# oleg-savchenko/jax_nbody_emulator_with_dj

Hardware: AMD Instinct MI355X
Metric: voxels/sec (disp+vel) on 512^3 box, ndiv=4 (higher is better)
Workload: dtype f32-equivalent: f16x3 split MFMA (3 f16 MFMAs per product, f32 accumulate)

## Files before the change

jax_nbody_emulator_with_dj_amd/csrc/nbe_engine_internal.h:

```cpp
#pragma once

#include "../../include/nbe.h"
#include "nbe_kernels.h"

#include <cmath>
#include <cstdarg>
#include <cstdio>
#include <cstdlib>
#include <cstring>
#include <algorithm>
#include <atomic>
#include <chrono>
#include <condition_variable>
#include <deque>
#include <functional>
#include <map>
#include <memory>
#include <mutex>
#include <string>
#include <thread>
#include <vector>

#pragma GCC visibility push(hidden)

// ... 184 lines not shown
    uint64_t graph_clock = 0, graph_replays = 0;
    int epoch = 0;
    hipEvent_t ev_g0 = nullptr, ev_g1 = nullptr;
    struct Probe {
        bool on = false, tile = false;
        int p[3] = {0, 0, 0}, nout = 0;
        int o[3] = {0, 0, 0};
        struct Slot { std::string name; int C, n, nw, level; int64_t off; };
        std::vector<Slot> slots;
        unsigned* bits = nullptr; int64_t words = 0;
        unsigned* count = nullptr;
    } probe;
    int* paths = nullptr;
    bool prof = false;
    std::vector<ProfEntry> prof_entries;
    struct Pending { int entry; hipEvent_t a, b; };
    std::vector<Pending> pending;
    std::vector<hipEvent_t> ev_pool;
};

struct HeadOut { void* disp; void* velo; int out_dtype; int OD, OH, OW, a0, a1, a2; float Dz, vel_fac; };

static constexpr int PIPE_EDGE = 32;

static constexpr int BRICK_H1 = 6, BRICK_H2 = 10;
static constexpr int BRICK_H0 = 4;

bool is_device_ptr(const void* p);
int require_ready(nbe_ctx* c);
int prepare_range(nbe_ctx* c, const float* dev_src, int64_t n, float Dz, const float* host_src = nullptr);
int check_range(nbe_ctx* c);

int planes_for(int C, int prec);
Tensor talloc(nbe_ctx* c, int C, int D, int H, int W);
Tensor tallocp(nbe_ctx* c, int C, int D, int Hi, int Wi, int pad);
void fill_halo(nbe_ctx* c, const Tensor& t);
void tfree(nbe_ctx* c, Tensor& t);
Tensor zview(const Tensor& t, int z0, int nz);
void set_org(Tensor& t, int z, int y, int x);
bool wino_f16_layer(int prec, bool vel, int cin_pad);
bool wino_env_off();
bool up8_launch(const nbe_ctx* c, const Layer& L, bool has_dx);
int run_conv(nbe_ctx* c, const Layer& L, const ConvLaunch& cl_in, bool has_dx);
const Layer* find_layer(nbe_ctx* c, const char* block, const char* layer);
bool block_fused(const nbe_ctx* c, const Layer* L1, int nres);
bool two_source_width(const nbe_ctx* c);
Tensor alloc_hidden(nbe_ctx* c, int cmid, int nz, const Tensor& x, bool fused);
int resblock_part(nbe_ctx* c, const char* name, const Tensor& x, const Tensor& h, const Tensor& s,
                  int js, int ns, int jh, int nh, bool has_dx, bool final_act, const int* zr, const Tensor* x2 = nullptr);
int resblock(nbe_ctx* c, const char* name, const Tensor& x, bool has_dx, bool final_act, int cout, int cmid, Tensor* out,
             Tensor* hidden_out = nullptr);
int down_conv(nbe_ctx* c, const Layer& L, const Tensor& x, Tensor& o, bool probe);
int downblock(nbe_ctx* c, const char* name, const Tensor& x, Tensor* out);
int upblock(nbe_ctx* c, const char* name, const Tensor& x, const Tensor& cat, int xcrop = 0, int g0 = -1);
void crop_into(nbe_ctx* c, const Tensor& src, int crop, const Tensor& dst, int cz = -1);
int check_dims(int D, int H, int W);
int check_dims_pyx(int D, int H, int W);
void run_head(nbe_ctx* c, const Tensor& y, const Tensor& xin, const HeadOut& h, int zoff);
int network(nbe_ctx* c, const Tensor& tin, Tensor* yout);
int network_stream(nbe_ctx* c, const Tensor& tin, const HeadOut& ho, int S);

PackedW layer_geometry(int prec, int kind, int cout, int cin);
bool packs_narrow(int prec, bool vel, const Layer& L);
bool packs_wino(int prec, bool vel, const Layer& L);
bool packs_wino_skip(int prec, bool vel, bool style, const Layer& L);
bool packs_stem(int prec, const Layer& L);
int alloc_wino(PackedW& pw);
int alloc_stem(PackedW& pw);
int wino_flag_round_trip(nbe_ctx* c, const std::function<void()>& packs);
void release_layer(Layer& L);
void free_layers(nbe_ctx* c);
int pack_wino(nbe_ctx* c);

unsigned host_absmax_bits(const float* x, int64_t n);
int pipe_input(nbe_ctx* c, const Tensor& tin, int t0, int t1, int look, float scale);
int pipe_output(nbe_ctx* c, int z, int n, int a1 = 0, int a2 = 0, int e1 = -1, int e2 = -1);
int ensure_workspace(nbe_ctx* c, int D, int H, int W);
int run_subbox(nbe_ctx* c, const float* box, int Db, int Hb, int Wb, int o0, int o1, int o2,
               int D, int H, int W, float Dz, float vel_fac, void* disp, void* velo, int out_dtype,
               int OD, int OH, int OW, int a0, int a1, int a2);
void drop_graphs(nbe_ctx* c);
int64_t plan_budget(nbe_ctx* c, int64_t reserve);
int choose_slab(nbe_ctx* c, int D, int H, int W, int64_t budget, int64_t* need_out, bool pyx = false, bool pz = false);

void brick_send(nbe_ctx* c, const Tensor& t, int in, int n, void* lo, void* hi);
// ... 13 lines not shown
```

jax_nbody_emulator_with_dj_amd/csrc/nbe_engine_net.cpp:

```cpp
#include "nbe_engine_internal.h"

int planes_for(int C, int prec) { return roundup(C, 16) / (prec == PREC_F16 ? 8 : 4); }

static Planes ws_planes(nbe_ctx* c, int G, int D, int H, int W, int64_t* off_out) {
    Planes p;
    p.G = G; p.D = D; p.H = H; p.W = W;
    p.pstride = (p.vox() + 63) & ~int64_t(63);
    const int64_t one = (int64_t)G * p.pstride * 16;
    const int64_t slack = ((int64_t)2 * H * W + 2 * W + 1024) * 16;
    const int64_t off = c->arena.alloc(one * (c->vel ? 2 : 1) + slack);
    *off_out = off;
    if (!c->dry) {
        p.x = (float*)(c->ws + off);
        p.dx = c->vel ? (float*)(c->ws + off + one) : nullptr;
    }
    return p;
}

Tensor talloc(nbe_ctx* c, int C, int D, int H, int W) {
    Tensor t;
    t.p = ws_planes(c, planes_for(C, c->prec), D, H, W, &t.off);
    const int gw = c->prec == PREC_F16 ? (C + 7) / 8 : c->prec == PREC_F16X3 ? 2 * ((C + 7) / 8) : (C + 3) / 4;
    if (!c->dry && t.off >= 0 && gw < t.p.G) {
        const size_t off = (size_t)gw * t.p.pstride * 4, bytes = (size_t)(t.p.G - gw) * t.p.pstride * 16;
        launch_zero(t.p.x + off, (int64_t)bytes, c->stream);
        if (t.p.dx) launch_zero(t.p.dx + off, (int64_t)bytes, c->stream);
    }
    return t;
}
Tensor tallocp(nbe_ctx* c, int C, int D, int Hi, int Wi, int pad) {
    Tensor t = talloc(c, C, D, Hi + 2 * pad, Wi + 2 * pad);
    t.pad = pad;
    return t;
}
static Planes inner(const Tensor& t) {
    Planes p = t.p;
    const int64_t sh = (int64_t)t.pad * (t.p.W + 1) * 4;
    if (p.x) p.x += sh;
    if (p.dx) p.dx += sh;
    return p;
}
void fill_halo(nbe_ctx* c, const Tensor& t) {
    if (t.pad > 0 && !c->dry) launch_fill_yx(t.p, t.pad, c->vel, c->stream);
}
void tfree(nbe_ctx* c, Tensor& t) { if (t.off >= 0) c->arena.release(t.off); t.off = -1; }
Tensor zview(const Tensor& t, int z0, int nz) {
    Tensor v = t;
    v.off = -1;
    const int64_t sh = (int64_t)z0 * t.p.H * t.p.W * 4;
    if (v.p.x) v.p.x += sh;
    if (v.p.dx) v.p.dx += sh;
    v.p.D = nz;
    v.org[0] += z0;
    return v;
}
static void org_conv(const Tensor& x, int nconv, int out[3]) {
    const int p = x.pad ? nconv : 0;
    out[0] = x.org[0]; out[1] = x.org[1] - p; out[2] = x.org[2] - p;
}
void set_org(Tensor& t, int z, int y, int x) { t.org[0] = z; t.org[1] = y; t.org[2] = x; }

static std::string conv_name(const PackedW& pw, bool vel, bool has_dx, bool g6 = false, bool up8 = false) {
    if (up8) return vel ? "up_h3<8 parities,vel,dx>" : "up_h3<8 parities,novel>";
    const char* m = pw.mode == MODE_FLAT3 ? "FLAT3" : pw.mode == MODE_FLAT1 ? "FLAT1" : "DOWN";
// ... 33 lines not shown
    int pe = -1; hipEvent_t ea = nullptr, eb = nullptr;
    if (c->prof) {
        std::string pn = cl.wino ? std::string(c->prec == PREC_F16 ? "conv_h1w<FLAT3,vel,dx>" : c->vel ? "conv_h3w<FLAT3,vel,dx>" : "conv_h3w<FLAT3,novel>")
                                 : conv_name(pw, c->vel, has_dx, g6, cl.set < 0);
        static const bool per_layer = getenv("NBE_PROF_LAYERS") && atoi(getenv("NBE_PROF_LAYERS")) == 1;
        if (per_layer) pn += " " + L.block + "/" + L.layer;
        pe = prof_entry(c, pn);
        ea = get_event(c); eb = get_event(c);
        (void)hipEventRecord(ea, c->stream);
    }
    if (launch_conv(pw, cl, c->vel, has_dx, c->stream))
        return fail("internal error: no kernel for layer %s/%s (mode %d, gauged %d, input tangent %d, crop offset %ld, output stride %d)",
                    L.block.c_str(), L.layer.c_str(), L.pw.mode, (int)g6, (int)has_dx, (long)cl.in_off, cl.osz);
    if (c->prof) {
        (void)hipEventRecord(eb, c->stream);
        c->pending.push_back({pe, ea, eb});
        const double nout = (double)cl.Dv * cl.Hv * cl.Wv * (cl.set < 0 ? 8.0 : 1.0);
        const int taps = L.kind == 0 ? 27 : L.kind == 2 ? 8 : 1;
        const double gemms = c->vel ? ((has_dx && !g6) ? 3.0 : 2.0) : 1.0;
        c->prof_entries[pe].flops += 2.0 * nout * L.cout * L.cin * taps * gemms;
        if (cl.skw) c->prof_entries[pe].flops += 2.0 * nout * L.cout * L.fskip->cin * (!c->vel ? 1.0 : (cl.flags & F_SKIP_NODX) ? 2.0 : 3.0);
        c->prof_entries[pe].launches += 1;
        if (c->pending.size() > 4096) prof_collect(c);
    }
    return 0;
}

const Layer* find_layer(nbe_ctx* c, const char* block, const char* layer) {
    auto it = c->layers.find(std::string(block) + "/" + layer);
    return it == c->layers.end() ? nullptr : &it->second;
}


static bool wino_only_fuse(const nbe_ctx* c) { return !c->vel || c->prec == PREC_F16; }
bool block_fused(const nbe_ctx* c, const Layer* L1, int nres) {
    return c->fuse && L1->fskip != nullptr && (!wino_only_fuse(c) || (!c->direct_z && !wino_env_off() && (nres & 1) == 0));
}

bool two_source_width(const nbe_ctx* c) { return c->mid % (c->prec == PREC_F16 ? 32 : 16) == 0; }

Tensor alloc_hidden(nbe_ctx* c, int cmid, int nz, const Tensor& x, bool fused) {
    const int pad = x.pad, sy = pad ? 0 : 2;
    if (fused && !pad) return talloc(c, cmid, nz, x.p.H, x.p.W);
    return tallocp(c, cmid, nz, x.p.H - 2 * pad - sy, x.p.W - 2 * pad - sy, pad);
}

int resblock_part(nbe_ctx* c, const char* name, const Tensor& x, const Tensor& h, const Tensor& s,
                         int js, int ns, int jh, int nh, bool has_dx, bool final_act, const int* zr, const Tensor* x2) {
    const Layer *Ls = find_layer(c, name, "skip"), *L0 = find_layer(c, name, "conv_0"), *L1 = find_layer(c, name, "conv_1");
    if (!Ls || !L0 || !L1) return fail("missing layers of block %s", name);
    const int H = x.p.H, W = x.p.W, pad = x.pad;
    const bool fused = block_fused(c, L1, ns);
    if (fused && (h.p.H != H || h.p.W != W)) return fail("internal: hidden tensor of fused block %s lacks the input's pitch", name);
    if (x2 && (!fused || x2->p.H != H || x2->p.W != W || x2->pad != pad)) return fail("internal: two-source input of block %s", name);
    const Tensor sv = zview(s, js, ns), hv = zview(h, jh, nh);
    const Tensor xs = zview(x, js, ns + 4);
    const int64_t sk_off = (2L * H + (pad ? pad : 2)) * W + (pad ? pad : 2);
    if (!fused) {
        ConvLaunch cl; cl.in = xs.p; cl.in_off = sk_off;
        cl.Dv = ns; cl.Hv = s.p.H - 2 * pad; cl.Wv = s.p.W - 2 * pad; cl.out = inner(sv); cl.flags = 0;
        if (run_conv(c, *Ls, cl, has_dx)) return 1;
    }
    int og[3];
    {
        ConvLaunch cl; cl.in = zview(x, jh, nh + 2).p; cl.Dv = nh; cl.Hv = H - 2; cl.Wv = W - 2; cl.out = inner(hv); cl.flags = F_ACT;
        if (x2) { cl.in2 = zview(*x2, jh, nh + 2).p; cl.csplit_ch = c->mid; }
        if (run_conv(c, *L0, cl, has_dx)) return 1;
        org_conv(x, 1, og); og[0] += jh;
        const int zh[3] = {zr ? zr[0] : 0, zr ? zr[1] + 2 : 0, zr ? zr[2] : 0};
        probe_act(c, *L0, cl.out, 0, og, cl.Dv, cl.Hv, cl.Wv, pad != 0, zr ? zh : nullptr);
    }
    fill_halo(c, hv);
    {
        ConvLaunch cl; cl.in = zview(h, js, ns + 2).p; cl.Dv = ns; cl.Hv = s.p.H - 2 * pad; cl.Wv = s.p.W - 2 * pad; cl.out = inner(sv);
        if (fused) { cl.sk = xs.p; cl.sk_off = sk_off; cl.skw = L1->pwn.w ? &Ls->pwn : &Ls->pw; cl.flags = (final_act ? F_ACT : 0) | (has_dx ? 0 : F_SKIP_NODX);
                     if (x2) { cl.sk2 = zview(*x2, js, ns + 4).p; cl.sk_split_ch = c->mid; } }
        else { cl.res = inner(sv); cl.flags = F_RES | (final_act ? F_ACT : 0); }
        if (run_conv(c, *L1, cl, true)) return 1;
        org_conv(x, 2, og); og[0] += js;
        if (final_act) probe_act(c, *L1, cl.out, 0, og, cl.Dv, cl.Hv, cl.Wv, pad != 0, zr);
    }
    fill_halo(c, sv);
    return 0;
}

int resblock(nbe_ctx* c, const char* name, const Tensor& x, bool has_dx, bool final_act, int cout, int cmid, Tensor* out,
                    Tensor* hidden_out) {
    const Layer* L1 = find_layer(c, name, "conv_1");
    if (!L1) return fail("missing layers of block %s", name);
    const int D = x.p.D, pad = x.pad;
    const int sy = pad ? 0 : 2;
    Tensor s = tallocp(c, cout, D - 4, x.p.H - 2 * pad - 2 * sy, x.p.W - 2 * pad - 2 * sy, pad);
    Tensor h = alloc_hidden(c, cmid, D - 2, x, block_fused(c, L1, D - 4));
    if (s.off < 0 || h.off < 0) return fail("workspace exhausted in block %s", name);
    if (resblock_part(c, name, x, h, s, 0, D - 4, 0, D - 2, has_dx, final_act, nullptr)) return 1;
    tfree(c, h);
    if (hidden_out) *hidden_out = h;
    int og[3];
    org_conv(x, 2, og);
    set_org(s, og[0], og[1], og[2]);
    *out = s;
    return 0;
}

static void carry_planes(nbe_ctx* c, const Tensor& t, int src, int dst, int n) {
    if (c->dry || n <= 0) return;
    launch_crop(zview(t, src, n).p, 0, zview(t, dst, n).p, 0, c->vel, c->stream, 0);
}

int down_conv(nbe_ctx* c, const Layer& L, const Tensor& x, Tensor& o, bool probe) {
    ConvLaunch cl; cl.in = inner(x); cl.Dv = o.p.D; cl.Hv = o.p.H; cl.Wv = o.p.W; cl.out = o.p; cl.flags = F_ACT;
    if (run_conv(c, L, cl, true)) return 1;
    set_org(o, x.org[0] / 2, x.org[1] / 2, x.org[2] / 2);
    if (probe) probe_act(c, L, cl.out, 0, o.org, cl.Dv, cl.Hv, cl.Wv, x.pad != 0);
    return 0;
}

int downblock(nbe_ctx* c, const char* name, const Tensor& x, Tensor* out) {
    const Layer* L = find_layer(c, name, "conv_0");
    if (!L) return fail("missing layer %s/conv_0", name);
    Tensor o = talloc(c, c->mid, x.p.D / 2, x.p.H / 2, x.p.W / 2);
    if (o.off < 0) return fail("workspace exhausted in %s", name);
    if (down_conv(c, *L, x, o, true)) return 1;
    *out = o;
    return 0;
}

static int mid_planes(const nbe_ctx* c) { return c->mid / (c->prec == PREC_F16 ? 8 : 4); }

int upblock(nbe_ctx* c, const char* name, const Tensor& x, const Tensor& cat, int xcrop, int g0) {
    const Layer* L = find_layer(c, name, "conv_0");
    if (!L) return fail("missing layer %s/conv_0", name);
    xcrop += x.pad;
    const int Hx = x.p.H - 2 * xcrop, Wx = x.p.W - 2 * xcrop;
    if (cat.p.D != 2 * x.p.D || cat.p.H - 2 * cat.pad != 2 * Hx || cat.p.W - 2 * cat.pad != 2 * Wx)
        return fail("internal: concat geometry mismatch in %s", name);
    const bool up8 = up8_launch(c, *L, true);
    const int out_g0 = g0 >= 0 ? g0 : mid_planes(c);
    for (int p = 0; p < (up8 ? 1 : 8); ++p) {
        ConvLaunch cl; cl.in = x.p; cl.in_off = ((int64_t)xcrop * x.p.W + xcrop);
        cl.Dv = x.p.D; cl.Hv = Hx; cl.Wv = Wx; cl.out = inner(cat);
        cl.out_g0 = out_g0; cl.osz = 2; cl.oz = (p >> 2) & 1; cl.oy = (p >> 1) & 1; cl.ox = p & 1;
        cl.flags = F_ACT; cl.set = up8 ? -1 : p;
        if (run_conv(c, *L, cl, true)) return 1;
    }
    const int xc = xcrop - x.pad;
    const int og[3] = {2 * x.org[0], 2 * (x.org[1] + xc), 2 * (x.org[2] + xc)};
    probe_act(c, *L, inner(cat), out_g0, og, 2 * x.p.D, 2 * Hx, 2 * Wx, cat.pad != 0);
// ... 4 lines not shown
    if (c->dry) return;
    Planes s = src.p; s.G = mid_planes(c);
    launch_crop(s, crop, dst.p, 0, c->vel, c->stream, cz);
}

int check_dims(int D, int H, int W) {
    const int v[3] = {D, H, W};
    for (int i = 0; i < 3; ++i)
        if (v[i] < 104 || v[i] % 8 != 0)
            return fail("input spatial size %d unsupported: each of (D,H,W) must be >= 104 and a multiple of 8 "
                        "(all-VALID U-Net with three 2x levels, receptive-field crop 48)", v[i]);
    return 0;
}

void run_head(nbe_ctx* c, const Tensor& y, const Tensor& xin, const HeadOut& h, int zoff) {
    if (c->dry) return;
    const float inv_s = 1.0f / c->act_scale;
    HeadScale hs;
    hs.k_disp = 6.0f * inv_s; hs.k_dy = h.vel_fac * 6.0f * inv_s; hs.k_x0 = h.vel_fac * 6.0f / h.Dz * inv_s;
    hs.bad = c->flags ? (int*)(c->flags + 1) : nullptr;
    launch_head(y.p, xin.p, 48, c->out_chan, hs, c->vel, h.disp, h.velo, h.out_dtype, h.OD, h.OH, h.OW,
                h.a0 + zoff, h.a1, h.a2, c->prec, c->stream, y.pad);
}

static int stream_encode(nbe_ctx* c, const Tensor& tin, const HeadOut& ho, int S, Tensor* skip0_out, Tensor* td_out) {
    const int m = c->mid, pad = tin.pad;
    const int D = tin.p.D, H = tin.p.H, W = tin.p.W;
    const int Hi = H - 2 * pad, Wi = W - 2 * pad;
    const int Y = D - 8;
    const bool zx = pad && c->zx;
    const bool pz = pad && (c->pz || zx);
    const int zlo = pz ? (zx ? 44 : 40) : 0, zhi = pz ? (zx ? Y - 44 : Y - 40) : Y;
    Tensor skip0 = pad ? tallocp(c, m, Y - 80, Hi, Wi, pad) : talloc(c, m, Y - 80, H - 88, W - 88);
    Tensor td = pad ? talloc(c, m, pz ? (D - 96) / 2 : Y / 2, Hi / 2, Wi / 2) : talloc(c, m, Y / 2, (H - 8) / 2, (W - 8) / 2);
    if (skip0.off < 0 || td.off < 0) return fail("workspace exhausted (level 0)");
    const Layer* Ld = find_layer(c, "down_l0", "conv_0");
    if (!Ld) return fail("missing layer down_l0/conv_0");
    const int sy = pad ? 0 : 2;
    const Layer* L00 = find_layer(c, "conv_l00", "conv_1");
    if (!L00) return fail("missing layer conv_l00/conv_1");
    Tensor h0 = alloc_hidden(c, m, S + 6, tin, block_fused(c, L00, S + 4)), a = tallocp(c, m, S + 4, Hi - 2 * sy, Wi - 2 * sy, pad);
    const Layer *L01 = find_layer(c, "conv_l01", "conv_1"), *Lr00 = find_layer(c, "conv_r00", "conv_1"), *Lr01 = find_layer(c, "conv_r01", "conv_1");
    if (!L01 || !Lr00 || !Lr01) return fail("missing conv_1 layers of the level-0 blocks");
    Tensor h1 = alloc_hidden(c, m, S + 2, a, block_fused(c, L01, S));
    Tensor y0r = pz ? Tensor() : tallocp(c, m, S, Hi - 4 * sy, Wi - 4 * sy, pad);
    if (h0.off < 0 || a.off < 0 || h1.off < 0 || (!pz && y0r.off < 0)) return fail("workspace exhausted (level-0 encoder slabs)");
    const int zr00[3] = {zlo, zhi + 4, pz ? D - 96 : 0}, zr01[3] = {zlo, zhi, pz ? D - 96 : 0};
    for (int z = zlo, n = 0; z < zhi; z += n) {
        n = std::min(((c->pipe.active || c->pipe.slabwise) && z == zlo) ? std::min(S, PIPE_EDGE) : S, zhi - z);
        const int n_next = std::min(S, zhi - (z + n));
        const bool first = z == zlo;
        Tensor y0 = pz ? zview(skip0, z - 40, n) : zview(y0r, 0, n);
        if ((c->pipe.active || c->pipe.slabwise) && !c->dry && pipe_input(c, tin, z, z + n + 8, n_next, ho.Dz / 6.0f * c->act_scale)) return 1;
        { int og[3]; org_conv(zview(tin, z, n + 8), 2, og); set_org(a, og[0], og[1], og[2]);
          org_conv(a, 2, og); set_org(y0, og[0], og[1], og[2]); }
        if (first) {
            if (resblock_part(c, "conv_l00", zview(tin, z, n + 8), h0, a, 0, n + 4, 0, n + 6, false, true, zr00)) return 1;
            if (resblock_part(c, "conv_l01", a, h1, y0, 0, n, 0, n + 2, true, true, zr01)) return 1;
        } else {
            if (resblock_part(c, "conv_l00", zview(tin, z, n + 8), h0, a, 4, n, 6, n, false, true, zr00)) return 1;
            if (resblock_part(c, "conv_l01", a, h1, y0, 0, n, 2, n, true, true, zr01)) return 1;
        }
        if (z + n < zhi) {
            carry_planes(c, h0, n, 0, 6);
            carry_planes(c, a, n, 0, 4);
            carry_planes(c, h1, n, 0, 2);
        }
        const int i0 = std::max(0, 40 - z), i1 = std::min(n, Y - 40 - z);
        if (!pz && i1 > i0) crop_into(c, y0, pad ? 0 : 40, zview(skip0, z + i0 - 40, i1 - i0), i0);
        {
            const int d0 = pz ? std::max(z, 44) : z, d1 = pz ? std::min(z + n, Y - 44) : z + n;
            if (d1 > d0) {
                const Tensor tv = zview(td, (d0 - (pz ? 44 : 0)) / 2, (d1 - d0) / 2);
                Tensor yv = zview(y0, d0 - z, d1 - d0);
                ConvLaunch cl; cl.in = inner(yv); cl.Dv = tv.p.D; cl.Hv = tv.p.H; cl.Wv = tv.p.W; cl.out = tv.p; cl.flags = F_ACT;
                if (run_conv(c, *Ld, cl, true)) return 1;
                const int og[3] = {yv.org[0] / 2, yv.org[1] / 2, yv.org[2] / 2};
                const int zd[3] = {22, 22 + (D - 96) / 2, pz ? (D - 96) / 2 : 0};
                probe_act(c, *Ld, cl.out, 0, og, cl.Dv, cl.Hv, cl.Wv, pad != 0, zd);
            }
        }
    }
    tfree(c, h0); tfree(c, a); tfree(c, h1);
    if (!pz) tfree(c, y0r);
    set_org(skip0, 0, pad ? 4 : 0, pad ? 4 : 0);
    set_org(td, pz ? 22 : 0, pad ? 22 : 0, pad ? 22 : 0);
    *skip0_out = skip0; *td_out = td;
    return 0;
}

static int stream_level1(nbe_ctx* c, int pad, bool pz, Tensor td, Tensor* cat1_out, Tensor* t_out) {
    const int m = c->mid;
    Tensor t = td;
    if (pad) {
        t = tallocp(c, m, td.p.D + (pz ? 44 : 0), td.p.H, td.p.W, 1);
        if (t.off < 0) return fail("workspace exhausted (level 1 input)");
        if (!c->dry) launch_wrap_pad(td.p, t.p, 1, c->vel, c->stream, pz ? 22 : 0);
        set_org(t, pz ? td.org[0] - 22 : td.org[0], td.org[1], td.org[2]);
        tfree(c, td);
    }

    Tensor y1, cat1;
    if (resblock(c, "conv_l1", t, true, true, m, m, &y1)) return 1;
    tfree(c, t);
    if (pad) {
        cat1 = tallocp(c, 2 * m, y1.p.D - 32, y1.p.H - 2, y1.p.W - 2, 1);
        if (cat1.off < 0) return fail("workspace exhausted (cat1)");
        crop_into(c, y1, 0, cat1, 16);
        set_org(cat1, y1.org[0], y1.org[1] - 16, y1.org[2] - 16);
        Tensor t2 = talloc(c, m, y1.p.D / 2, (y1.p.H - 2) / 2, (y1.p.W - 2) / 2);
        const Layer* Ld1 = find_layer(c, "down_l1", "conv_0");
        if (t2.off < 0 || !Ld1) return fail("workspace exhausted or missing layer (down_l1)");
        if (down_conv(c, *Ld1, y1, t2, true)) return 1;
        t = talloc(c, m, t2.p.D, t2.p.H + 20, t2.p.W + 20);
        if (t.off < 0) return fail("workspace exhausted (level 2 input)");
        if (!c->dry) launch_wrap_pad(t2.p, t.p, 10, c->vel, c->stream, 0);
        set_org(t, t2.org[0], t2.org[1] - 10, t2.org[2] - 10);
        tfree(c, t2);
    } else {
        cat1 = talloc(c, 2 * m, y1.p.D - 32, y1.p.H - 32, y1.p.W - 32);
        if (cat1.off < 0) return fail("workspace exhausted (cat1)");
        crop_into(c, y1, 16, cat1);
        if (downblock(c, "down_l1", y1, &t)) return 1;
    }
    tfree(c, y1);
    *cat1_out = cat1; *t_out = t;
    return 0;
}

static int lower_levels(nbe_ctx* c, Tensor t, Tensor cat1, Tensor* r_out) {
    const int m = c->mid;
    Tensor y2, cat2, r;
    if (resblock(c, "conv_l2", t, true, true, m, m, &y2)) return 1;
    tfree(c, t);
    cat2 = talloc(c, 2 * m, y2.p.D - 8, y2.p.H - 8, y2.p.W - 8);
    if (cat2.off < 0) return fail("workspace exhausted (cat2)");
    crop_into(c, y2, 4, cat2);
    if (downblock(c, "down_l2", y2, &t)) return 1;
    tfree(c, y2);

    c->direct_z = true;
    const int rc = resblock(c, "conv_c", t, true, true, m, m, &r);
    c->direct_z = false;
    if (rc) return 1;
    tfree(c, t);

    if (upblock(c, "up_r2", r, cat2)) return 1;
    tfree(c, r);
    if (resblock(c, "conv_r2", cat2, true, true, m, 2 * m, &r)) return 1;
    tfree(c, cat2);

    if (upblock(c, "up_r1", r, cat1, cat1.pad ? 2 : 0)) return 1;
    fill_halo(c, cat1);
    tfree(c, r);
    if (resblock(c, "conv_r1", cat1, true, true, m, 2 * m, r_out)) return 1;
    tfree(c, cat1);
    return 0;
}

int network(nbe_ctx* c, const Tensor& tin, Tensor* yout) {
    const int m = c->mid;
    Tensor a, y0, t, cat0, cat1, r;
    if (resblock(c, "conv_l00", tin, false, true, m, m, &a)) return 1;
    if (resblock(c, "conv_l01", a, true, true, m, m, &y0)) return 1;
    tfree(c, a);
    cat0 = talloc(c, 2 * m, y0.p.D - 80, y0.p.H - 80, y0.p.W - 80);
    if (cat0.off < 0) return fail("workspace exhausted (cat0)");
    crop_into(c, y0, 40, cat0);
    if (downblock(c, "down_l0", y0, &t)) return 1;
    tfree(c, y0);

    if (stream_level1(c, 0, false, t, &cat1, &t)) return 1;
    if (lower_levels(c, t, cat1, &r)) return 1;

    if (upblock(c, "up_r0", r, cat0)) return 1;
    tfree(c, r);
    if (resblock(c, "conv_r00", cat0, true, true, m, 2 * m, &r)) return 1;
    tfree(c, cat0);

    if (resblock(c, "conv_r01", r, true, false, c->out_chan, m, yout)) return 1;
    tfree(c, r);
    return 0;
}

static int stream_tail(nbe_ctx* c, const Tensor& tin, const HeadOut& ho, int S, Tensor skip0, Tensor cat1, Tensor t) {
    const int m = c->mid, pad = tin.pad;
    const int sy = pad ? 0 : 2;
    const Layer *Lr00 = find_layer(c, "conv_r00", "conv_1"), *Lr01 = find_layer(c, "conv_r01", "conv_1");
    if (!Lr00 || !Lr01) return fail("missing conv_1 layers of the level-0 blocks");
    Tensor r;
    if (lower_levels(c, t, cat1, &r)) return 1;
    if (2 * r.p.D != skip0.p.D || 2 * (r.p.H - 2 * r.pad) != skip0.p.H - 2 * pad || 2 * (r.p.W - 2 * r.pad) != skip0.p.W - 2 * pad)
        return fail("internal: level-0 concat geometry mismatch");

    if (pad && c->zx && !c->dry && c->bio.skip_recv_lo) {
        if (c->bio.skip_ready) HIPCHK(hipStreamWaitEvent(c->stream, c->bio.skip_ready, 0));
        brick_recv(c, skip0, c->bio.skip_recv_lo, c->bio.skip_recv_hi, BRICK_H0, skip0, 0);
    }
    const int Yo = skip0.p.D - 8;
    const int Hs = skip0.p.H - 2 * pad, Ws = skip0.p.W - 2 * pad;
    const bool two = block_fused(c, Lr00, S + 4) && two_source_width(c);
    Tensor cat = tallocp(c, two ? m : 2 * m, S + 8, Hs, Ws, pad), hq = alloc_hidden(c, 2 * m, S + 6, cat, block_fused(c, Lr00, S + 4));
    Tensor q = tallocp(c, m, S + 4, Hs - 2 * sy, Ws - 2 * sy, pad), hy = alloc_hidden(c, m, S + 2, q, block_fused(c, Lr01, S));
    Tensor y = tallocp(c, c->out_chan, S, Hs - 4 * sy, Ws - 4 * sy, pad);
    if (cat.off < 0 || hq.off < 0 || q.off < 0 || hy.off < 0 || y.off < 0) return fail("workspace exhausted (level-0 decoder slabs)");
    for (int z = 0, n = 0; z < Yo; z += n) {
        n = std::min(S, Yo - z);
        if (c->pipe.active && c->pipe.out_async && Yo - z > PIPE_EDGE && Yo - z - n < PIPE_EDGE)
            n = Yo - z - PIPE_EDGE;
        const bool first = z == 0;
        const int c0 = first ? 0 : 8, cn = first ? n + 8 : n;
        set_org(cat, skip0.org[0] + z, skip0.org[1], skip0.org[2]);
        { int og[3]; org_conv(cat, 2, og); set_org(q, og[0], og[1], og[2]); }
        if (!two && !c->dry) launch_crop(zview(skip0, z + c0, cn).p, 0, zview(cat, c0, cn).p, 0, c->vel, c->stream, 0);
        if (upblock(c, "up_r0", zview(r, (z + c0) / 2, cn / 2), zview(cat, c0, cn), 0, two ? 0 : -1)) return 1;
        fill_halo(c, zview(cat, c0, cn));
        const Tensor sk = two ? zview(skip0, z, std::min(S + 8, skip0.p.D - z)) : cat;
        const Tensor* up2 = two ? &cat : nullptr;
        if (first) {
            if (resblock_part(c, "conv_r00", sk, hq, q, 0, n + 4, 0, n + 6, true, true, nullptr, up2)) return 1;
            if (resblock_part(c, "conv_r01", q, hy, y, 0, n, 0, n + 2, true, false, nullptr)) return 1;
        } else {
            if (resblock_part(c, "conv_r00", sk, hq, q, 4, n, 6, n, true, true, nullptr, up2)) return 1;
            if (resblock_part(c, "conv_r01", q, hy, y, 0, n, 2, n, true, false, nullptr)) return 1;
        }
        if (z + n < Yo) {
            carry_planes(c, cat, n, 0, 8);
            carry_planes(c, hq, n, 0, 6);
            carry_planes(c, q, n, 0, 4);
            carry_planes(c, hy, n, 0, 2);
        }
        run_head(c, zview(y, 0, n), zview(tin, z, n + 96), ho, z);
        if (c->pipe.active && c->pipe.out_async && !c->dry && pipe_output(c, z, n)) return 1;
        if (c->prog && !c->dry && z + n < Yo)
            c->prog->post(c->pipe.active && c->pipe.out_async ? c->down_stream : c->stream,
                          c->prog_k * 1000 + (int)(1000L * (z + n) / Yo), c->prog_n * 1000);
    }
    tfree(c, cat); tfree(c, hq); tfree(c, q); tfree(c, hy); tfree(c, y);
    tfree(c, r); tfree(c, skip0);
    return 0;
}

static void stash_arena(nbe_ctx* c) { c->sst.blks = c->arena.blks; c->sst.high = c->arena.high; }

int network_stream(nbe_ctx* c, const Tensor& tin, const HeadOut& ho, int S) {
    auto& st = c->sst;
    const int pad = tin.pad;
    const bool zx = pad && c->zx;
    if (c->phase >= 2) {
        if (!st.valid || st.stage != c->phase - 1) return fail("brick calls out of order (encode, interior, exchange, finish) or the context was used in between");
        c->arena.blks = st.blks; c->arena.high = st.high;
    }
    if (c->phase <= 1) {
        if (stream_encode(c, tin, ho, S, &st.skip0, &st.td)) return 1;
        st.tin = tin; st.S = S;
        if (c->phase == 1) {
            brick_send(c, st.td, 0, BRICK_H1, c->bio.send_lo, c->bio.send_hi);
            brick_send(c, st.skip0, BRICK_H0, BRICK_H0, c->bio.skip_send_lo, c->bio.skip_send_hi);
            st.valid = true; st.stage = 1; stash_arena(c);
            return 0;
        }
    }
    if (!zx) {
        Tensor cat1, t;
        if (stream_level1(c, pad, pad && c->pz, st.td, &cat1, &t)) return 1;
        return stream_tail(c, tin, ho, S, st.skip0, cat1, t);
    }
    if (c->phase == 0 || c->phase == 2) {
        if (brick_interior(c, st)) return 1;
        if (c->phase == 2) { st.stage = 2; stash_arena(c); return 0; }
    }
    if (c->phase == 0 || c->phase == 3) {
        if (brick_edges(c, st)) return 1;
        if (c->phase == 3) { st.stage = 3; stash_arena(c); return 0; }
    }
    Tensor t;
    if (brick_level2(c, st, &t)) return 1;
    st.valid = false;
    return stream_tail(c, st.tin, ho, st.S, st.skip0, st.cat1, t);
}

int check_dims_pyx(int D, int H, int W) {
    if (D < 104 || D % 8 != 0) return fail("input depth %d unsupported: must be >= 104 and a multiple of 8", D);
    const int v[2] = {H - 2, W - 2};
    for (int i = 0; i < 2; ++i)
        if (v[i] < 48 || v[i] % 8 != 0) return fail("periodic extent %d unsupported: must be >= 48 and a multiple of 8", v[i]);
    return 0;
}
```

jax_nbody_emulator_with_dj_amd/csrc/nbe_kernels.hip:

```cpp

#include "nbe_kernels_internal.h"
#include <algorithm>
#include <cstdint>
#include <cstdio>
#include <cstdlib>

namespace nbe {

#define LDS_AS NBE_LDS_AS
#define GLB_AS NBE_GLB_AS

extern __shared__ __attribute__((aligned(16))) f32x4 lds_dyn[];

template <int MODE, bool VEL, bool HAS_DX, int NI, bool G6 = false>
__global__ __launch_bounds__(256, 2) void conv_mfma_kernel(ConvKArgs a) {
    constexpr int CK = mode_ck(MODE), GL = CK / 4, TAPS = mode_taps(MODE);
    constexpr int COUT_T = 32 * NI;
    constexpr int XV = (MODE == MODE_FLAT3) ? 320 : 256;
    constexpr int WP = TAPS * GL * COUT_T;
    constexpr int XP = GL * XV;
    constexpr bool DX = VEL && HAS_DX;
    constexpr bool DWT = VEL && !G6;
    static_assert(!G6 || (DX && MODE == MODE_FLAT3), "gauged form: 3x3x3 layers with an input tangent");
    constexpr int OFF_W = 0, OFF_DW = WP, OFF_X = OFF_DW + (DWT ? WP : 0), OFF_DXX = OFF_X + XP;
// ... 90 lines not shown
                }
#pragma unroll
                for (int r = 0; r < 4; ++r) {
#pragma unroll
                    for (int it = 0; it < NI; ++it) {
#pragma unroll
                        for (int jt = 0; jt < 2; ++jt) {
                            accy[it][jt] = __builtin_amdgcn_mfma_f32_32x32x2f32(wv[it][r], xv[jt][r], accy[it][jt], 0, 0, 0);
                            if (DWT) accd[it][jt] = __builtin_amdgcn_mfma_f32_32x32x2f32(dwv[it][r], xv[jt][r], accd[it][jt], 0, 0, 0);
                            if (DX) accd[it][jt] = __builtin_amdgcn_mfma_f32_32x32x2f32(wv[it][r], dxv[jt][r], accd[it][jt], 0, 0, 0);
                        }
                    }
                }
            }
        }
    };

    issue(0, 0);
    __syncthreads();
    for (int s = 0; s < nstage; ++s) {
        if (s + 1 < nstage) issue(s + 1, (s + 1) & 1);
        compute(s & 1);
        __syncthreads();
    }

    const bool act = a.flags & F_ACT, res = a.flags & F_RES;
#pragma unroll
    for (int jt = 0; jt < 2; ++jt) {
        const long q = q0 + wave * 64 + 32 * jt + li;
        bool valid = q < a.Q;
        long o;
        if (MODE == MODE_DOWN) {
            o = q;
        } else {
            const int z = (int)(q / HW), rem = (int)(q - (long)z * HW);
            const int yy = rem / a.W, xx = rem - yy * a.W;
            valid = valid && xx < a.Wv && yy < a.Hv && z < a.Dv;
            o = ((long)(z * a.osz + a.oz) * a.Ho + (yy * a.osz + a.oy)) * a.Wo + (xx * a.osz + a.ox);
        }
        if (!valid) continue;
#pragma unroll
        for (int it = 0; it < NI; ++it) {
#pragma unroll
            for (int k = 0; k < 4; ++k) {
                const int cgl = 8 * it + 2 * k + lh;
                const int cg = ct * (COUT_T / 4) + cgl;
                if (cg >= a.cout_groups) continue;
                const f32x4 bv = *(const f32x4*)(a.bias + cg * 4);
                f32x4 v, dv;
#pragma unroll
                for (int e = 0; e < 4; ++e) { v[e] = accy[it][jt][4 * k + e] + bv[e]; dv[e] = accd[it][jt][4 * k + e]; }
                if (G6) {
                    const f32x4 be = *(const f32x4*)(a.beta + cg * 4);
#pragma unroll
                    for (int e = 0; e < 4; ++e) dv[e] += be[e] * accy[it][jt][4 * k + e];
                }
                if (res) {
                    const long ro = ((long)cg * a.res_pstride + o) * 4;
                    const f32x4 rv = *(const f32x4*)(a.r + ro);
                    v += rv;
                    if (VEL) { const f32x4 drv = *(const f32x4*)(a.dr + ro); dv += drv; }
                }
                if (act) {
#pragma unroll
                    for (int e = 0; e < 4; ++e) {
                        if (VEL) dv[e] = v[e] > 0.f ? dv[e] : 0.01f * dv[e];
// ... 495 lines not shown
```

jax_nbody_emulator_with_dj_amd/csrc/nbe_kernels_h3.hip:

```cpp

#include "nbe_kernels_internal.h"
#include <cstdlib>
#include <cstdio>
#include <algorithm>

#ifndef NBE_DBG
#define NBE_DBG 0
#endif

namespace nbe {

extern __shared__ __attribute__((aligned(16))) f32x4 lds_h3[];

__device__ __forceinline__ void split4(const f32x4 v, half4& hi, half4& lo) {
#pragma unroll
    for (int e = 0; e < 4; ++e) {
        hi[e] = (_Float16)v[e];
        lo[e] = (_Float16)__builtin_fmaf((float)hi[e], -H3_SCALE, v[e] * H3_SCALE);
    }
}
__device__ __forceinline__ f32x4 join4(const half4 hi, const half4 lo) {
    f32x4 v;
#pragma unroll
    for (int e = 0; e < 4; ++e) v[e] = (float)hi[e] + (float)lo[e] * H3_INV;
// ... 232 lines not shown
        const bool pw = s + 1 < nstage, px = s + 1 < nstage;
        const long xoff2 = px ? seg_offset(s + 1) : 0;
        const int ring2 = ring ^ 1;
        const half8* wb = (const half8*)(lds + (s & 1) * WB);
        const half8* xb = (const half8*)(lds + XRING + ring * XB);
        Ops o0, o1;
        load_ops(wb, xb, o0);
        __builtin_amdgcn_sched_barrier(0);
#pragma unroll
        for (int i = 0; i < 18; ++i) {
            mfma1(o0, i);
            if (i & 1) {
                const int t = i >> 1;
                if (t < NWS) { if (pw) dma_w(t, s + 1); }
                else if (t - NWS < NXS) { if (px) dma_x(t - NWS, xoff2, ring2); }
                __builtin_amdgcn_sched_barrier(0);
            }
        }
        __builtin_amdgcn_sched_barrier(0);
        __builtin_amdgcn_sched_barrier(0);
        wait_all();
        barrier();
        ring = ring == 1 ? 0 : ring + 1;
    }

    long o[2];
    bool ok[2];
#pragma unroll
    for (int jt = 0; jt < 2; ++jt) {
        const long q = q0 + jq * 64 + 32 * jt + li;
        ok[jt] = q < a.Q;
        if (MODE == MODE_DOWN) {
            o[jt] = q;
        } else {
            const int z = (int)(q / HW), rem = (int)(q - (long)z * HW);
            const int yy = rem / a.W, xx = rem - yy * a.W;
            ok[jt] = ok[jt] && xx < a.Wv && yy < a.Hv && z < a.Dv;
            o[jt] = ((long)(z * a.osz + a.oz) * a.Ho + (yy * a.osz + a.oy)) * a.Wo + (xx * a.osz + a.ox);
        }
        if (!ok[jt]) o[jt] = 0;
    }
    h3_store2<VEL, SPLIT>(a, ct, it, lh, o, ok, ym, yc, dm, dc);
}

constexpr int UP_XV = 256;
constexpr int UP_MAXCH = 4;
template <bool SPLIT> struct UpGeom {
    static constexpr int UN = SPLIT ? 4 : 2;
    static constexpr int XC = 2 * UN * UP_XV;
    static constexpr int WS = 2 * 2 * UN * 64;
    static constexpr int WBASE = UP_MAXCH * XC;
    static constexpr int LDS_UNITS = WBASE + 2 * WS;
};

template <bool SPLIT, bool VEL = true>
__global__ __launch_bounds__(512, 2) void up_h3_kernel(ConvKArgs a) {
    constexpr int UN = UpGeom<SPLIT>::UN, UP_XC = UpGeom<SPLIT>::XC, UP_WS = UpGeom<SPLIT>::WS, UP_WBASE = UpGeom<SPLIT>::WBASE;
    constexpr int PS = SPLIT ? 2 : 1;
    f32x4* lds = lds_h3;
    const half8* L8 = (const half8*)lds_h3;
    const int tid = threadIdx.x;
    const int lane = tid & 63;
    const int wave = __builtin_amdgcn_readfirstlane(tid >> 6);
    const int li = lane & 31, lh = lane >> 5;
    const int it = wave & 1, jq = wave >> 1;
    const int tile = xcd_tile(blockIdx.x, a.ntiles);
// ... 1702 lines not shown
```

Before: 100.7 million.

## Write downsample outputs directly into padded tensors and skip intermediate wrap-pad copies

The level-0 and level-1 downsample convolutions now write straight into the interior of pre-padded tensors, which carry z context planes. Halos are then filled in place with fill_halo and wrap_z plane carries. This replaces the separate wrap_pad allocation and copy kernels. Level 1 can also feed the conv_r1 block as two sources without building the cat1 concat, and the final output tensor skips zeroing its unused channel groups. The down-mode store kernels gain a strided output index path. The changes add index arithmetic and more complex geometry bookkeeping that could hide off-by-one errors.

```diff
diff --git a/jax_nbody_emulator_with_dj_amd/csrc/nbe_engine_internal.h b/jax_nbody_emulator_with_dj_amd/csrc/nbe_engine_internal.h
--- a/jax_nbody_emulator_with_dj_amd/csrc/nbe_engine_internal.h
+++ b/jax_nbody_emulator_with_dj_amd/csrc/nbe_engine_internal.h
@@ -240,8 +240,8 @@
 int check_range(nbe_ctx* c);
 
 int planes_for(int C, int prec);
-Tensor talloc(nbe_ctx* c, int C, int D, int H, int W);
-Tensor tallocp(nbe_ctx* c, int C, int D, int Hi, int Wi, int pad);
+Tensor talloc(nbe_ctx* c, int C, int D, int H, int W, bool zero_rest = true);
+Tensor tallocp(nbe_ctx* c, int C, int D, int Hi, int Wi, int pad, bool zero_rest = true);
 void fill_halo(nbe_ctx* c, const Tensor& t);
 void tfree(nbe_ctx* c, Tensor& t);
 Tensor zview(const Tensor& t, int z0, int nz);
@@ -255,10 +255,11 @@
 bool two_source_width(const nbe_ctx* c);
 Tensor alloc_hidden(nbe_ctx* c, int cmid, int nz, const Tensor& x, bool fused);
 int resblock_part(nbe_ctx* c, const char* name, const Tensor& x, const Tensor& h, const Tensor& s,
-                  int js, int ns, int jh, int nh, bool has_dx, bool final_act, const int* zr, const Tensor* x2 = nullptr);
+                  int js, int ns, int jh, int nh, bool has_dx, bool final_act, const int* zr, const Tensor* x2 = nullptr,
+                  bool halo_s = true);
 int resblock(nbe_ctx* c, const char* name, const Tensor& x, bool has_dx, bool final_act, int cout, int cmid, Tensor* out,
-             Tensor* hidden_out = nullptr);
-int down_conv(nbe_ctx* c, const Layer& L, const Tensor& x, Tensor& o, bool probe);
+             Tensor* hidden_out = nullptr, const int* zr = nullptr, const Tensor* x2 = nullptr);
+int down_conv(nbe_ctx* c, const Layer& L, const Tensor& x, Tensor& o, bool probe, const int* zr = nullptr);
 int downblock(nbe_ctx* c, const char* name, const Tensor& x, Tensor* out);
 int upblock(nbe_ctx* c, const char* name, const Tensor& x, const Tensor& cat, int xcrop = 0, int g0 = -1);
 void crop_into(nbe_ctx* c, const Tensor& src, int crop, const Tensor& dst, int cz = -1);
diff --git a/jax_nbody_emulator_with_dj_amd/csrc/nbe_engine_net.cpp b/jax_nbody_emulator_with_dj_amd/csrc/nbe_engine_net.cpp
--- a/jax_nbody_emulator_with_dj_amd/csrc/nbe_engine_net.cpp
+++ b/jax_nbody_emulator_with_dj_amd/csrc/nbe_engine_net.cpp
@@ -17,19 +17,19 @@
     return p;
 }
 
-Tensor talloc(nbe_ctx* c, int C, int D, int H, int W) {
+Tensor talloc(nbe_ctx* c, int C, int D, int H, int W, bool zero_rest) {
     Tensor t;
     t.p = ws_planes(c, planes_for(C, c->prec), D, H, W, &t.off);
     const int gw = c->prec == PREC_F16 ? (C + 7) / 8 : c->prec == PREC_F16X3 ? 2 * ((C + 7) / 8) : (C + 3) / 4;
-    if (!c->dry && t.off >= 0 && gw < t.p.G) {
+    if (zero_rest && !c->dry && t.off >= 0 && gw < t.p.G) {
         const size_t off = (size_t)gw * t.p.pstride * 4, bytes = (size_t)(t.p.G - gw) * t.p.pstride * 16;
         launch_zero(t.p.x + off, (int64_t)bytes, c->stream);
         if (t.p.dx) launch_zero(t.p.dx + off, (int64_t)bytes, c->stream);
     }
     return t;
 }
-Tensor tallocp(nbe_ctx* c, int C, int D, int Hi, int Wi, int pad) {
-    Tensor t = talloc(c, C, D, Hi + 2 * pad, Wi + 2 * pad);
+Tensor tallocp(nbe_ctx* c, int C, int D, int Hi, int Wi, int pad, bool zero_rest) {
+    Tensor t = talloc(c, C, D, Hi + 2 * pad, Wi + 2 * pad, zero_rest);
     t.pad = pad;
     return t;
 }
@@ -129,6 +129,8 @@
 }
 
 
+static constexpr int L1_CTX = BRICK_H1, L2_CTX = BRICK_H2;
+
 static bool wino_only_fuse(const nbe_ctx* c) { return !c->vel || c->prec == PREC_F16; }
 bool block_fused(const nbe_ctx* c, const Layer* L1, int nres) {
     return c->fuse && L1->fskip != nullptr && (!wino_only_fuse(c) || (!c->direct_z && !wino_env_off() && (nres & 1) == 0));
@@ -143,7 +145,7 @@
 }
 
 int resblock_part(nbe_ctx* c, const char* name, const Tensor& x, const Tensor& h, const Tensor& s,
-                         int js, int ns, int jh, int nh, bool has_dx, bool final_act, const int* zr, const Tensor* x2) {
+                         int js, int ns, int jh, int nh, bool has_dx, bool final_act, const int* zr, const Tensor* x2, bool halo_s) {
     const Layer *Ls = find_layer(c, name, "skip"), *L0 = find_layer(c, name, "conv_0"), *L1 = find_layer(c, name, "conv_1");
     if (!Ls || !L0 || !L1) return fail("missing layers of block %s", name);
     const int H = x.p.H, W = x.p.W, pad = x.pad;
@@ -177,12 +179,12 @@
         org_conv(x, 2, og); og[0] += js;
         if (final_act) probe_act(c, *L1, cl.out, 0, og, cl.Dv, cl.Hv, cl.Wv, pad != 0, zr);
     }
-    fill_halo(c, sv);
+    if (halo_s) fill_halo(c, sv);
     return 0;
 }
 
 int resblock(nbe_ctx* c, const char* name, const Tensor& x, bool has_dx, bool final_act, int cout, int cmid, Tensor* out,
-                    Tensor* hidden_out) {
+                    Tensor* hidden_out, const int* zr, const Tensor* x2) {
     const Layer* L1 = find_layer(c, name, "conv_1");
     if (!L1) return fail("missing layers of block %s", name);
     const int D = x.p.D, pad = x.pad;
@@ -190,7 +192,7 @@
     Tensor s = tallocp(c, cout, D - 4, x.p.H - 2 * pad - 2 * sy, x.p.W - 2 * pad - 2 * sy, pad);
     Tensor h = alloc_hidden(c, cmid, D - 2, x, block_fused(c, L1, D - 4));
     if (s.off < 0 || h.off < 0) return fail("workspace exhausted in block %s", name);
-    if (resblock_part(c, name, x, h, s, 0, D - 4, 0, D - 2, has_dx, final_act, nullptr)) return 1;
+    if (resblock_part(c, name, x, h, s, 0, D - 4, 0, D - 2, has_dx, final_act, zr, x2)) return 1;
     tfree(c, h);
     if (hidden_out) *hidden_out = h;
     int og[3];
@@ -205,12 +207,21 @@
     launch_crop(zview(t, src, n).p, 0, zview(t, dst, n).p, 0, c->vel, c->stream, 0);
 }
 
-int down_conv(nbe_ctx* c, const Layer& L, const Tensor& x, Tensor& o, bool probe) {
-    ConvLaunch cl; cl.in = inner(x); cl.Dv = o.p.D; cl.Hv = o.p.H; cl.Wv = o.p.W; cl.out = o.p; cl.flags = F_ACT;
+int down_conv(nbe_ctx* c, const Layer& L, const Tensor& x, Tensor& o, bool probe, const int* zr) {
+    ConvLaunch cl; cl.in = inner(x); cl.Dv = o.p.D; cl.Hv = o.p.H - 2 * o.pad; cl.Wv = o.p.W - 2 * o.pad; cl.out = inner(o); cl.flags = F_ACT;
     if (run_conv(c, L, cl, true)) return 1;
     set_org(o, x.org[0] / 2, x.org[1] / 2, x.org[2] / 2);
-    if (probe) probe_act(c, L, cl.out, 0, o.org, cl.Dv, cl.Hv, cl.Wv, x.pad != 0);
-    return 0;
+    if (probe) probe_act(c, L, cl.out, 0, o.org, cl.Dv, cl.Hv, cl.Wv, x.pad != 0, zr);
+    return 0;
+}
+
+static void wrap_z(nbe_ctx* c, const Tensor& t, int cz) {
+    const int own = t.p.D - 2 * cz;
+    for (int done = 0; done < cz; done += own) {
+        const int n = std::min(own, cz - done);
+        carry_planes(c, t, cz - done - n + own, cz - done - n, n);
+        carry_planes(c, t, cz + done, cz + own + done, n);
+    }
 }
 
 int downblock(nbe_ctx* c, const char* name, const Tensor& x, Tensor* out) {
@@ -281,7 +292,9 @@
     const bool pz = pad && (c->pz || zx);
     const int zlo = pz ? (zx ? 44 : 40) : 0, zhi = pz ? (zx ? Y - 44 : Y - 40) : Y;
     Tensor skip0 = pad ? tallocp(c, m, Y - 80, Hi, Wi, pad) : talloc(c, m, Y - 80, H - 88, W - 88);
-    Tensor td = pad ? talloc(c, m, pz ? (D - 96) / 2 : Y / 2, Hi / 2, Wi / 2) : talloc(c, m, Y / 2, (H - 8) / 2, (W - 8) / 2);
+    const int cz1 = (pz && !zx) ? L1_CTX : 0, dpad = (pad && !zx) ? 1 : 0;
+    const int D1 = pz ? (D - 96) / 2 : Y / 2;
+    Tensor td = pad ? tallocp(c, m, D1 + 2 * cz1, Hi / 2, Wi / 2, dpad) : talloc(c, m, Y / 2, (H - 8) / 2, (W - 8) / 2);
     if (skip0.off < 0 || td.off < 0) return fail("workspace exhausted (level 0)");
     const Layer* Ld = find_layer(c, "down_l0", "conv_0");
     if (!Ld) return fail("missing layer down_l0/conv_0");
@@ -320,9 +333,9 @@
         {
             const int d0 = pz ? std::max(z, 44) : z, d1 = pz ? std::min(z + n, Y - 44) : z + n;
             if (d1 > d0) {
-                const Tensor tv = zview(td, (d0 - (pz ? 44 : 0)) / 2, (d1 - d0) / 2);
+                const Tensor tv = zview(td, cz1 + (d0 - (pz ? 44 : 0)) / 2, (d1 - d0) / 2);
                 Tensor yv = zview(y0, d0 - z, d1 - d0);
-                ConvLaunch cl; cl.in = inner(yv); cl.Dv = tv.p.D; cl.Hv = tv.p.H; cl.Wv = tv.p.W; cl.out = tv.p; cl.flags = F_ACT;
+                ConvLaunch cl; cl.in = inner(yv); cl.Dv = tv.p.D; cl.Hv = tv.p.H - 2 * dpad; cl.Wv = tv.p.W - 2 * dpad; cl.out = inner(tv); cl.flags = F_ACT;
                 if (run_conv(c, *Ld, cl, true)) return 1;
                 const int og[3] = {yv.org[0] / 2, yv.org[1] / 2, yv.org[2] / 2};
                 const int zd[3] = {22, 22 + (D - 96) / 2, pz ? (D - 96) / 2 : 0};
@@ -333,51 +346,59 @@
     tfree(c, h0); tfree(c, a); tfree(c, h1);
     if (!pz) tfree(c, y0r);
     set_org(skip0, 0, pad ? 4 : 0, pad ? 4 : 0);
-    set_org(td, pz ? 22 : 0, pad ? 22 : 0, pad ? 22 : 0);
+    set_org(td, pz ? 22 - cz1 : 0, pad ? 22 : 0, pad ? 22 : 0);
     *skip0_out = skip0; *td_out = td;
     return 0;
 }
 
-static int stream_level1(nbe_ctx* c, int pad, bool pz, Tensor td, Tensor* cat1_out, Tensor* t_out) {
+static int stream_level1(nbe_ctx* c, int pad, bool pz, Tensor td, Tensor* cat1_out, Tensor* y1_out, Tensor* t_out) {
     const int m = c->mid;
-    Tensor t = td;
-    if (pad) {
-        t = tallocp(c, m, td.p.D + (pz ? 44 : 0), td.p.H, td.p.W, 1);
-        if (t.off < 0) return fail("workspace exhausted (level 1 input)");
-        if (!c->dry) launch_wrap_pad(td.p, t.p, 1, c->vel, c->stream, pz ? 22 : 0);
-        set_org(t, pz ? td.org[0] - 22 : td.org[0], td.org[1], td.org[2]);
-        tfree(c, td);
-    }
-
-    Tensor y1, cat1;
-    if (resblock(c, "conv_l1", t, true, true, m, m, &y1)) return 1;
-    tfree(c, t);
-    if (pad) {
-        cat1 = tallocp(c, 2 * m, y1.p.D - 32, y1.p.H - 2, y1.p.W - 2, 1);
-        if (cat1.off < 0) return fail("workspace exhausted (cat1)");
-        crop_into(c, y1, 0, cat1, 16);
-        set_org(cat1, y1.org[0], y1.org[1] - 16, y1.org[2] - 16);
-        Tensor t2 = talloc(c, m, y1.p.D / 2, (y1.p.H - 2) / 2, (y1.p.W - 2) / 2);
-        const Layer* Ld1 = find_layer(c, "down_l1", "conv_0");
-        if (t2.off < 0 || !Ld1) return fail("workspace exhausted or missing layer (down_l1)");
-        if (down_conv(c, *Ld1, y1, t2, true)) return 1;
-        t = talloc(c, m, t2.p.D, t2.p.H + 20, t2.p.W + 20);
-        if (t.off < 0) return fail("workspace exhausted (level 2 input)");
-        if (!c->dry) launch_wrap_pad(t2.p, t.p, 10, c->vel, c->stream, 0);
-        set_org(t, t2.org[0], t2.org[1] - 10, t2.org[2] - 10);
-        tfree(c, t2);
-    } else {
+    Tensor t = td, y1, cat1;
+    *y1_out = Tensor();
+    if (!pad) {
+        if (resblock(c, "conv_l1", t, true, true, m, m, &y1)) return 1;
+        tfree(c, t);
         cat1 = talloc(c, 2 * m, y1.p.D - 32, y1.p.H - 32, y1.p.W - 32);
         if (cat1.off < 0) return fail("workspace exhausted (cat1)");
         crop_into(c, y1, 16, cat1);
         if (downblock(c, "down_l1", y1, &t)) return 1;
-    }
-    tfree(c, y1);
+        tfree(c, y1);
+        *cat1_out = cat1; *t_out = t;
+        return 0;
+    }
+    const int cz1 = pz ? L1_CTX : 0, cz2 = pz ? L2_CTX : 0;
+    fill_halo(c, zview(t, cz1, t.p.D - 2 * cz1));
+    wrap_z(c, t, cz1);
+    const int zr1[3] = {t.org[0], t.org[0] + t.p.D - 4, t.p.D - 2 * cz1};
+    if (resblock(c, "conv_l1", t, true, true, m, m, &y1, nullptr, pz ? zr1 : nullptr)) return 1;
+    tfree(c, t);
+
+    const int zc = pz ? 0 : 16;
+    const Layer *Lr1 = find_layer(c, "conv_r1", "conv_1"), *Ld1 = find_layer(c, "down_l1", "conv_0");
+    if (!Lr1 || !Ld1) return fail("missing layer conv_r1/conv_1 or down_l1/conv_0");
+    const bool two = block_fused(c, Lr1, y1.p.D - 2 * zc - 4) && two_source_width(c);
+    if (!two) {
+        cat1 = tallocp(c, 2 * m, y1.p.D - 2 * zc, y1.p.H - 2, y1.p.W - 2, 1);
+        if (cat1.off < 0) return fail("workspace exhausted (cat1)");
+        crop_into(c, y1, 0, cat1, zc);
+        set_org(cat1, y1.org[0] + zc - 16, y1.org[1] - 16, y1.org[2] - 16);
+    }
+    Tensor y1d = pz ? zview(y1, 4, y1.p.D - 8) : y1;
+    t = talloc(c, m, y1d.p.D / 2 + 2 * cz2, (y1.p.H - 2) / 2 + 2 * L2_CTX, (y1.p.W - 2) / 2 + 2 * L2_CTX);
+    if (t.off < 0) return fail("workspace exhausted (level 2 input)");
+    Tensor tp = zview(t, cz2, y1d.p.D / 2);
+    tp.pad = L2_CTX;
+    const int zd[3] = {y1d.org[0] / 2, y1d.org[0] / 2 + tp.p.D, tp.p.D};
+    if (down_conv(c, *Ld1, y1d, tp, true, pz ? zd : nullptr)) return 1;
+    fill_halo(c, tp);
+    wrap_z(c, t, cz2);
+    set_org(t, tp.org[0] - cz2, tp.org[1] - L2_CTX, tp.org[2] - L2_CTX);
+    if (two) *y1_out = y1; else tfree(c, y1);
     *cat1_out = cat1; *t_out = t;
     return 0;
 }
 
-static int lower_levels(nbe_ctx* c, Tensor t, Tensor cat1, Tensor* r_out) {
+static int lower_levels(nbe_ctx* c, Tensor t, Tensor cat1, Tensor y1, Tensor* r_out) {
     const int m = c->mid;
     Tensor y2, cat2, r;
     if (resblock(c, "conv_l2", t, true, true, m, m, &y2)) return 1;
@@ -399,17 +420,27 @@
     if (resblock(c, "conv_r2", cat2, true, true, m, 2 * m, &r)) return 1;
     tfree(c, cat2);
 
-    if (upblock(c, "up_r1", r, cat1, cat1.pad ? 2 : 0)) return 1;
+    const bool two = y1.off >= 0;
+    Tensor sk;
+    if (two) {
+        cat1 = tallocp(c, m, 2 * r.p.D, y1.p.H - 2, y1.p.W - 2, 1);
+        if (cat1.off < 0) return fail("workspace exhausted (up_r1)");
+        sk = zview(y1, (y1.p.D - 2 * r.p.D) / 2, 2 * r.p.D);
+        set_org(sk, sk.org[0] - 16, y1.org[1] - 16, y1.org[2] - 16);
+        set_org(cat1, sk.org[0], sk.org[1], sk.org[2]);
+    }
+    if (upblock(c, "up_r1", r, cat1, cat1.pad ? 2 : 0, two ? 0 : -1)) return 1;
     fill_halo(c, cat1);
     tfree(c, r);
-    if (resblock(c, "conv_r1", cat1, true, true, m, 2 * m, r_out)) return 1;
+    if (resblock(c, "conv_r1", two ? sk : cat1, true, true, m, 2 * m, r_out, nullptr, nullptr, two ? &cat1 : nullptr)) return 1;
     tfree(c, cat1);
+    if (two) tfree(c, y1);
     return 0;
 }
 
 int network(nbe_ctx* c, const Tensor& tin, Tensor* yout) {
     const int m = c->mid;
-    Tensor a, y0, t, cat0, cat1, r;
+    Tensor a, y0, t, cat0, cat1, y1, r;
     if (resblock(c, "conv_l00", tin, false, true, m, m, &a)) return 1;
     if (resblock(c, "conv_l01", a, true, true, m, m, &y0)) return 1;
     tfree(c, a);
@@ -419,8 +450,8 @@
     if (downblock(c, "down_l0", y0, &t)) return 1;
     tfree(c, y0);
 
-    if (stream_level1(c, 0, false, t, &cat1, &t)) return 1;
-    if (lower_levels(c, t, cat1, &r)) return 1;
+    if (stream_level1(c, 0, false, t, &cat1, &y1, &t)) return 1;
+    if (lower_levels(c, t, cat1, y1, &r)) return 1;
 
     if (upblock(c, "up_r0", r, cat0)) return 1;
     tfree(c, r);
@@ -432,13 +463,13 @@
     return 0;
 }
 
-static int stream_tail(nbe_ctx* c, const Tensor& tin, const HeadOut& ho, int S, Tensor skip0, Tensor cat1, Tensor t) {
+static int stream_tail(nbe_ctx* c, const Tensor& tin, const HeadOut& ho, int S, Tensor skip0, Tensor cat1, Tensor y1, Tensor t) {
     const int m = c->mid, pad = tin.pad;
     const int sy = pad ? 0 : 2;
     const Layer *Lr00 = find_layer(c, "conv_r00", "conv_1"), *Lr01 = find_layer(c, "conv_r01", "conv_1");
     if (!Lr00 || !Lr01) return fail("missing conv_1 layers of the level-0 blocks");
     Tensor r;
-    if (lower_levels(c, t, cat1, &r)) return 1;
+    if (lower_levels(c, t, cat1, y1, &r)) return 1;
     if (2 * r.p.D != skip0.p.D || 2 * (r.p.H - 2 * r.pad) != skip0.p.H - 2 * pad || 2 * (r.p.W - 2 * r.pad) != skip0.p.W - 2 * pad)
         return fail("internal: level-0 concat geometry mismatch");
 
@@ -451,7 +482,7 @@
     const bool two = block_fused(c, Lr00, S + 4) && two_source_width(c);
     Tensor cat = tallocp(c, two ? m : 2 * m, S + 8, Hs, Ws, pad), hq = alloc_hidden(c, 2 * m, S + 6, cat, block_fused(c, Lr00, S + 4));
     Tensor q = tallocp(c, m, S + 4, Hs - 2 * sy, Ws - 2 * sy, pad), hy = alloc_hidden(c, m, S + 2, q, block_fused(c, Lr01, S));
-    Tensor y = tallocp(c, c->out_chan, S, Hs - 4 * sy, Ws - 4 * sy, pad);
+    Tensor y = tallocp(c, c->out_chan, S, Hs - 4 * sy, Ws - 4 * sy, pad, false);
     if (cat.off < 0 || hq.off < 0 || q.off < 0 || hy.off < 0 || y.off < 0) return fail("workspace exhausted (level-0 decoder slabs)");
     for (int z = 0, n = 0; z < Yo; z += n) {
         n = std::min(S, Yo - z);
@@ -468,10 +499,10 @@
         const Tensor* up2 = two ? &cat : nullptr;
         if (first) {
             if (resblock_part(c, "conv_r00", sk, hq, q, 0, n + 4, 0, n + 6, true, true, nullptr, up2)) return 1;
-            if (resblock_part(c, "conv_r01", q, hy, y, 0, n, 0, n + 2, true, false, nullptr)) return 1;
+            if (resblock_part(c, "conv_r01", q, hy, y, 0, n, 0, n + 2, true, false, nullptr, nullptr, false)) return 1;
         } else {
             if (resblock_part(c, "conv_r00", sk, hq, q, 4, n, 6, n, true, true, nullptr, up2)) return 1;
-            if (resblock_part(c, "conv_r01", q, hy, y, 0, n, 2, n, true, false, nullptr)) return 1;
+            if (resblock_part(c, "conv_r01", q, hy, y, 0, n, 2, n, true, false, nullptr, nullptr, false)) return 1;
         }
         if (z + n < Yo) {
             carry_planes(c, cat, n, 0, 8);
@@ -511,9 +542,9 @@
         }
     }
     if (!zx) {
-        Tensor cat1, t;
-        if (stream_level1(c, pad, pad && c->pz, st.td, &cat1, &t)) return 1;
-        return stream_tail(c, tin, ho, S, st.skip0, cat1, t);
+        Tensor cat1, y1, t;
+        if (stream_level1(c, pad, pad && c->pz, st.td, &cat1, &y1, &t)) return 1;
+        return stream_tail(c, tin, ho, S, st.skip0, cat1, y1, t);
     }
     if (c->phase == 0 || c->phase == 2) {
         if (brick_interior(c, st)) return 1;
@@ -526,7 +557,7 @@
     Tensor t;
     if (brick_level2(c, st, &t)) return 1;
     st.valid = false;
-    return stream_tail(c, st.tin, ho, st.S, st.skip0, st.cat1, t);
+    return stream_tail(c, st.tin, ho, st.S, st.skip0, st.cat1, Tensor(), t);
 }
 
 int check_dims_pyx(int D, int H, int W) {
diff --git a/jax_nbody_emulator_with_dj_amd/csrc/nbe_kernels.hip b/jax_nbody_emulator_with_dj_amd/csrc/nbe_kernels.hip
--- a/jax_nbody_emulator_with_dj_amd/csrc/nbe_kernels.hip
+++ b/jax_nbody_emulator_with_dj_amd/csrc/nbe_kernels.hip
@@ -146,6 +146,12 @@
         long o;
         if (MODE == MODE_DOWN) {
             o = q;
+            if (a.Ho != a.Hv || a.Wo != a.Wv) {
+                const int hw = a.Hv * a.Wv;
+                const int z = (int)(q / hw), rem = (int)(q - (long)z * hw);
+                const int yy = rem / a.Wv, xx = rem - yy * a.Wv;
+                o = ((long)z * a.Ho + yy) * a.Wo + xx;
+            }
         } else {
             const int z = (int)(q / HW), rem = (int)(q - (long)z * HW);
             const int yy = rem / a.W, xx = rem - yy * a.W;
diff --git a/jax_nbody_emulator_with_dj_amd/csrc/nbe_kernels_h3.hip b/jax_nbody_emulator_with_dj_amd/csrc/nbe_kernels_h3.hip
--- a/jax_nbody_emulator_with_dj_amd/csrc/nbe_kernels_h3.hip
+++ b/jax_nbody_emulator_with_dj_amd/csrc/nbe_kernels_h3.hip
@@ -288,6 +288,12 @@
         ok[jt] = q < a.Q;
         if (MODE == MODE_DOWN) {
             o[jt] = q;
+            if (a.Ho != a.Hv || a.Wo != a.Wv) {
+                const int hw = a.Hv * a.Wv;
+                const int z = (int)(q / hw), rem = (int)(q - (long)z * hw);
+                const int yy = rem / a.Wv, xx = rem - yy * a.Wv;
+                o[jt] = ((long)z * a.Ho + yy) * a.Wo + xx;
+            }
         } else {
             const int z = (int)(q / HW), rem = (int)(q - (long)z * HW);
             const int yy = rem / a.W, xx = rem - yy * a.W;
```

Measured after the change: 102.0 million (median of 6 runs). 1.01x the previous value.
